# dfm/emcee

Hardware: NVIDIA H100
Metric: walker-steps/sec (nwalkers x iters / s) (higher is better)
Workload: dtype f64

## Files before the change

emcee_b200/_lib.py:

```python

import ctypes as C
import os

import numpy as np

__all__ = ["lib", "Engine", "Chain", "EngineError", "device_count", "LIB_PATH", "EbMove", "DeviceRows", "DeviceArray"]

HERE = os.path.dirname(os.path.abspath(__file__))
LIB_PATH = os.environ.get("EMCEE_B200_LIB") or os.path.join(HERE, "libemcee_b200.so")

EB_OK = 0
EB_ERR_INVALID = -1
EB_ERR_CUDA = -2
EB_ERR_COMM = -3
EB_ERR_STATE = -4
EB_ERR_UNSUPPORTED = -5
EB_ERR_NOMEM = -6
EB_ERR_CALLBACK = -7
EB_ERR_NAN_LOGPROB = -10
EB_ERR_INF_PARAM = -11
EB_ERR_NAN_PARAM = -12
EB_ERR_FEW_WALKERS = -13
EB_ERR_NAN_INITIAL = -14
EB_ERR_SINGULAR = -15
# ... 150 lines not shown
    "eb_trace_best": (C.c_int, [C.c_void_p, _dp, _dp, C.POINTER(C.c_uint64), C.POINTER(C.c_uint64)]),
    "eb_reservoir_config": (C.c_int, [C.c_void_p, C.c_uint64, C.c_uint64]),
    "eb_reservoir_count": (C.c_int, [C.c_void_p, C.POINTER(C.c_uint64), C.POINTER(C.c_uint64)]),
    "eb_reservoir_read": (C.c_int, [C.c_void_p, _dp, _dp, C.POINTER(C.c_uint64), C.POINTER(C.c_int64)]),
    "eb_reservoir_read_to": (C.c_int, [C.c_void_p, C.c_void_p, C.c_void_p, C.POINTER(C.c_uint64),
                                       C.POINTER(C.c_int64)]),
    "eb_walkers_gram": (C.c_int, [C.c_void_p, _dp, C.c_size_t, _dp, C.POINTER(C.c_int)]),
    "eb_autocorr": (C.c_int, [C.c_void_p, _dp, C.c_size_t, C.c_size_t, C.c_size_t, _dp]),
    "eb_last_step_timing": (C.c_int, [C.c_void_p, _dp, C.POINTER(C.c_uint64)]),
    "eb_debug_taps": (
        C.c_int,
        [C.c_void_p, C.POINTER(C.c_int64), _dp, _dp, C.POINTER(C.c_int64), C.POINTER(C.c_int64)],
    ),
    "eb_set_option": (C.c_int, [C.c_void_p, C.c_char_p, C.c_int64]),
    "eb_debug_timeline": (C.c_int, [C.c_void_p, C.POINTER(C.c_int64), C.c_size_t, C.POINTER(C.c_size_t)]),
    "eb_last_kernel_name": (C.c_char_p, [C.c_void_p]),
    "eb_last_kernel_variant": (C.c_char_p, [C.c_void_p]),
    "eb_microbench": (C.c_int, [C.c_int, C.c_int, _dp]),
    "eb_host_alloc": (C.c_int, [C.c_size_t, C.POINTER(C.c_void_p)]),
    "eb_host_free": (C.c_int, [C.c_void_p]),
    "eb_comm_id": (C.c_int, [C.c_char_p]),
    "eb_comm_init": (C.c_int, [C.c_void_p, C.c_char_p, C.c_int, C.c_int, C.c_int]),
    "eb_comm_export": (C.c_int, [C.c_void_p, C.c_char_p]),
    "eb_comm_import": (C.c_int, [C.c_void_p, C.c_char_p]),
    "eb_comm_probe": (C.c_int, [C.c_void_p, C.c_int, C.c_int, _dp]),
    "eb_device_alloc": (C.c_int, [C.c_int, C.c_size_t, C.POINTER(C.c_void_p)]),
    "eb_device_free": (C.c_int, [C.c_int, C.c_void_p]),
    "eb_device_copy": (C.c_int, [C.c_int, C.c_void_p, C.c_void_p, C.c_int64, C.c_int64, C.c_int64, C.c_uint64]),
    "eb_set_state_from": (C.c_int, [C.c_void_p, C.c_void_p, C.c_int64, C.c_void_p, C.c_int64, C.c_uint64]),
    "eb_get_state_to": (C.c_int, [C.c_void_p, C.c_void_p, C.c_void_p]),
# ... 1050 lines not shown
        self._check(
            lib().eb_debug_taps(
                self._h, partners.ctypes.data_as(i64), _as_dp(scalar), _as_dp(u),
                active.ctypes.data_as(i64), C.byref(cnt),
            )
        )
        k = int(cnt.value)
        return dict(partners=partners[:, :k], scalar=scalar[:k], u_accept=u[:k], active=active[:k])

    def debug_timeline(self):
        buf = np.zeros(1 << 21, dtype=np.int64)
        n = C.c_size_t()
        self._check(lib().eb_debug_timeline(self._h, buf.ctypes.data_as(C.POINTER(C.c_int64)), buf.size, C.byref(n)))
        return buf[: n.value].reshape(-1, 8, 8, 10)

    @staticmethod
    def comm_id():
        buf = C.create_string_buffer(EB_COMM_ID_BYTES)
        rc = lib().eb_comm_id(buf)
        if rc != EB_OK:
            raise EngineError("eb_comm_id failed (is libnccl.so.2 loadable?)")
        return buf.raw

    def comm_init(self, comm_id, rank, nranks, mode=EB_COMM_ALLGATHER):
        assert len(comm_id) == EB_COMM_ID_BYTES
        self._check(lib().eb_comm_init(self._h, comm_id, int(rank), int(nranks), int(mode)))

    def comm_export(self):
        buf = C.create_string_buffer(EB_IPC_BLOB_BYTES)
        self._check(lib().eb_comm_export(self._h, buf))
# ... 10 lines not shown
```

emcee_b200/csrc/capi.cu:

```cuda
#include <math.h>
#include <stdio.h>
#include <stdlib.h>
#include <string.h>

#include <algorithm>
#include <cmath>
#include <string>
#include <vector>

#include "chain_map.h"
#include "context.h"

static thread_local std::string g_create_err;

static const char* const MSG_BLOBS_WITH_LOG_PROB =
    "If you start sampling with a given log_prob, you also need to provide the current list of blobs at that "
    "position.";

int check_status(eb_ctx* c) {
  int f = *c->status_host;
  c->gm_unchecked = false;
  const unsigned long long g = graph_errors(c) ? *c->graph_err_host : 0ull;
  if (g != 0) {
    *c->graph_err_host = 0;
// ... 107 lines not shown
  cudaStream_t st = c->st.get();
  const size_t nd = (size_t)nwalkers * (size_t)ndim;
  CREATE_CK(dev_alloc(c->coords, nd * sizeof(double) + MAX_RANKS * sizeof(unsigned)));
  CREATE_CK(dev_alloc(c->logp, (size_t)nwalkers * sizeof(double)));
  CREATE_CK(dev_alloc(c->accepted, (size_t)nwalkers));
  CREATE_CK(dev_alloc(c->nacc, (size_t)nwalkers * sizeof(unsigned long long)));
  CREATE_CK(dev_alloc(c->status_dev, sizeof(int)));
  CREATE_CK(host_alloc(c->status_host, sizeof(int)));
  *c->status_host = 0;
  CREATE_CK(cudaMemsetAsync(c->status_dev.get(), 0, sizeof(int), st));
  CREATE_CK(cudaMemsetAsync(c->accepted.get(), 0, (size_t)nwalkers, st));
  CREATE_CK(cudaMemsetAsync(c->nacc.get(), 0, (size_t)nwalkers * sizeof(unsigned long long), st));
  size_t cap = (64u << 20) / ((size_t)nwalkers * sizeof(int32_t));
  cap = std::max<size_t>(1, std::min<size_t>(cap, 512));
  c->table_cap = cap;
  CREATE_CK(dev_alloc(c->order, cap * (size_t)nwalkers * sizeof(int32_t)));
  CREATE_CK(dev_alloc(c->info_dev, cap * sizeof(StepInfo)));
  CREATE_CK(host_alloc(c->info_host, cap * sizeof(StepInfo)));
  CREATE_CK(dev_alloc(c->descs_dev, cap * MAX_SPLITS * sizeof(HalfDesc)));
  CREATE_CK(host_alloc(c->descs_host, cap * MAX_SPLITS * sizeof(HalfDesc)));
  CREATE_CK(dev_alloc(c->gbar, sizeof(unsigned long long)));
  CREATE_CK(cudaMemsetAsync(c->gbar.get(), 0, sizeof(unsigned long long), st));
  CREATE_CK(cudaStreamSynchronize(st));
  *out = c.release();
  return EB_OK;
}

int eb_destroy(eb_ctx* c) {
  if (!c) return EB_OK;
  NOT_IN_CALLBACK(c);
// ... 1732 lines not shown
    c->local_first = (int)std::max<int64_t>(0, std::min<int64_t>(value, 2));
    return EB_OK;
  }
  if (!strcmp(name, "pdl")) {
    c->pdl = (int)std::max<int64_t>(0, std::min<int64_t>(value, 2));
    return EB_OK;
  }
  if (!strcmp(name, "moments_every")) {
    if (value < 0) FAIL(c, EB_ERR_INVALID, "moments_every must be >= 0");
    return moments_config(c, (uint64_t)value);
  }
  if (!strcmp(name, "tma_rows")) {
    c->allow_tma = (int)std::max<int64_t>(0, std::min<int64_t>(value, 2));
    return EB_OK;
  }
  if (!strcmp(name, "dense_dmma")) {
    c->allow_dmma = value != 0;
    return EB_OK;
  }
  FAIL(c, EB_ERR_INVALID, "eb_set_option: unknown option '%s'", name);
}

int eb_debug_timeline(eb_ctx* c, int64_t* out, size_t capacity, size_t* written) {
  if (!c || !out) return EB_ERR_INVALID;
  NOT_IN_CALLBACK(c);
  if (!c->timeline) FAIL(c, EB_ERR_STATE, "eb_debug_timeline: enable with eb_set_option(\"dmma_timeline\", 1)");
  CK(c, cudaSetDevice(c->device));
  const size_t n = (size_t)c->sm_count * 8 * TL_TILES * TL_EVENTS;
  if (capacity < n) FAIL(c, EB_ERR_INVALID, "eb_debug_timeline: need room for %zu values", n);
  CK(c, cudaMemcpy(out, c->timeline.get(), n * sizeof(long long), cudaMemcpyDeviceToHost));
// ... 167 lines not shown
```

emcee_b200/csrc/context.h:

```cpp
#pragma once

#include <stdio.h>

#include <string>
#include <vector>

#include "comm.h"
#include "engine.cuh"
#include "hist_bins.h"
#include "owners.h"
#include "reservoir_plan.h"
#include "trace_sum.h"

using namespace eb;


struct ChainSeg {
  DevPtr<double> x;
  DevPtr<double> lp;
};

struct eb_chain {
  int device = 0;
  int sm_count = 0;
// ... 30 lines not shown
  DevPtr<double> model_chol;
  DevPtr<double> model_box;
  bool have_model = false, have_state = false;

  DevPtr<int32_t> order;
  size_t table_cap = 0;
  DevPtr<StepInfo> info_dev;
  HostPtr<StepInfo> info_host;
  DevPtr<HalfDesc> descs_dev;
  HostPtr<HalfDesc> descs_host;
  DevPtr<unsigned long long> gbar;
  unsigned long long gbar_count = 0;
  uint64_t tbl_seed = 0, tbl_step0 = 0;
  size_t tbl_n = 0;
  std::vector<StepInfo> tbl_info;

  DevPtr<double> scratch_x;
  DevPtr<double> scratch_lp;
  size_t scratch_rows = 0;

  HostPtr<double> stage[2];
  HostPtr<uint8_t> stage_acc[2];
  EventPtr stage_ev[2];

  bool debug = false;
  DevPtr<int64_t> tap_partners;
  DevPtr<double> tap_scalar;
  DevPtr<double> tap_u;
  DevPtr<int64_t> tap_active;
  int64_t tap_count = 0;
// ... 170 lines not shown
      cudaGetLastError();                   \
      FAIL(ctx, EB_ERR_NOMEM, __VA_ARGS__); \
    }                                       \
  } while (0)

inline bool graph_mode(const eb_ctx* c) { return c->model.kind == MODEL_EXTERNAL && c->cb_where == EB_CALLBACK_GRAPH; }
inline bool proposal_graphs(const eb_ctx* c) {
  for (const eb_ctx::ProposalGraphs& p : c->prop_graphs)
    if (!p.graphs.empty()) return true;
  return false;
}
inline const eb_ctx::ProposalGraphs* slot_graphs(const eb_ctx* c, size_t slot) {
  return slot < c->prop_graphs.size() && !c->prop_graphs[slot].graphs.empty() ? &c->prop_graphs[slot] : nullptr;
}
inline bool graph_errors(const eb_ctx* c) { return graph_mode(c) || proposal_graphs(c); }
int check_status(eb_ctx* c);
int fetch_status(eb_ctx* c);
int enqueue_status_read(eb_ctx* c);
int run_callback(eb_ctx* c, const double* x, int64_t m, double* lp, bool scan_x);
void owned_rows(const eb_ctx* c, int64_t& r0, int64_t& r1);
int sync_replicas(eb_ctx* c);
```

emcee_b200/csrc/dense_dmma.cu:

```cuda
#include <math.h>

#include "draws.cuh"
#include "engine.cuh"
#include "tma.cuh"

namespace eb {

namespace {

constexpr int DMMA_CONSUMERS = 8;
constexpr int DMMA_THREADS = 64 * DMMA_CONSUMERS;
constexpr int NI = 2;
constexpr int DMMA_PRODUCER_REGS = 64;
constexpr int DMMA_CONSUMER_REGS = 192;
static_assert((DMMA_THREADS / 2) * (DMMA_PRODUCER_REGS + DMMA_CONSUMER_REGS) <= 65536, "register file of one SM");
__host__ __device__ constexpr bool dmma_rebalance(int KB, bool HAS_MEAN, bool BOUNDED) {
  return !BOUNDED && (KB >= 15 || (HAS_MEAN && KB >= 11));
}

__device__ __forceinline__ void dmma1688(double (&c)[4], double2 a01, double2 a23, double b0, double b1) {
  asm volatile(
      "mma.sync.aligned.m16n8k8.row.col.f64.f64.f64.f64 {%0,%1,%2,%3}, {%4,%5,%6,%7}, {%8,%9}, {%0,%1,%2,%3};"
      : "+d"(c[0]), "+d"(c[1]), "+d"(c[2]), "+d"(c[3])
      : "d"(a01.x), "d"(a01.y), "d"(a23.x), "d"(a23.y), "d"(b0), "d"(b1));
// ... 116 lines not shown
  double* sL = reinterpret_cast<double*>(smem_raw);
  double* sMu = sL + SL::off_mu;
  double* sSlots = sL + SL::off_slots;
  TileMeta* sMeta = reinterpret_cast<TileMeta*>(sL + SL::off_meta);
  uint64_t* bars = reinterpret_cast<uint64_t*>(smem_raw + SL::off_bars_bytes);
  volatile int* sAbort = reinterpret_cast<volatile int*>(smem_raw + SL::off_abort_bytes);
  volatile int* sPeers = sAbort + 1;
  int32_t* sInbox = reinterpret_cast<int32_t*>(smem_raw + SL::off_inbox_bytes);
  uint64_t* barL = bars;
  uint64_t* barFull = bars + 1;
  uint64_t* barReady = bars + 1 + DMMA_CONSUMERS;
  uint64_t* barFree = bars + 1 + 2 * DMMA_CONSUMERS;

  const int tid = threadIdx.x, lane = tid & 31, warp = tid >> 5;
  const bool is_producer = warp >= DMMA_CONSUMERS;
  const int pair = is_producer ? warp - DMMA_CONSUMERS : warp;
  const int g = lane >> 2, t = lane & 3;

  if (tid == 0) {
    *sAbort = 0;
    *sPeers = 0;
    mbar_init(barL, 1);
    for (int c = 0; c < DMMA_CONSUMERS; ++c) {
      mbar_init(barFull + c, 1);
      mbar_init(barReady + c, 1);
      mbar_init(barFree + c, 1);
    }
    asm volatile("fence.mbarrier_init.release.cluster;" ::: "memory");
  }
  if (HAS_MEAN)
    for (int k = tid; k < D; k += DMMA_THREADS) sMu[k] = a.model.params[k];
  __syncthreads();

  const int tstride = (int)gridDim.x * DMMA_CONSUMERS;
  const int tile0 = (int)blockIdx.x + (int)gridDim.x * pair;
  double* slot = sSlots + (size_t)pair * SL::slot_doubles;
  double* myS = slot + (size_t)g * RS + 2 * t;
  double* myC = myS + 8 * RS;
  TileMeta* meta = sMeta + 2 * pair;
  const bool multi = a.p2p_peer_flags != nullptr;
  unsigned k = 0;

  constexpr bool REBALANCE = dmma_rebalance(KB, HAS_MEAN, BOUNDED);
  if (is_producer) {
    if constexpr (REBALANCE) asm volatile("setmaxnreg.dec.sync.aligned.u32 %0;" ::"n"(DMMA_PRODUCER_REGS));
    const long long t_entry_p = clock64();
    long long* tlp = (TIMELINE && lane == 0)
                         ? a.timeline + ((size_t)blockIdx.x * DMMA_CONSUMERS + pair) * TL_TILES * TL_EVENTS : nullptr;
    const double dm1 = (double)a.D - 1.0;
    const int row = lane & 7;
    struct Prep {
      int32_t w, wp;
      double zz, factor, log_u, lp_old;
      bool valid, remote;
    };
    for (int h = 0; h < nhalf; ++h) {
      const HalfDesc d = (h == 0) ? d0 : descs[h];
      const int32_t* order = a.order + (size_t)d.order_step * a.N;
      const int2 rg = a.range ? a.range[(size_t)d.order_step * MAX_SPLITS + d.split] : make_int2(0, d.a_count);
      const int i_lo = rg.x, i_hi = rg.y;
      const int ntiles = (int)(((int64_t)i_hi - i_lo + 7) >> 3);
      const int64_t Nc = a.N - d.a_count;
      const int32_t* aperm = a.aperm ? a.aperm + (size_t)d.order_step * a.N + d.a_start : nullptr;
      auto prep = [&](int tile, bool with_lp) -> Prep {
        Prep p;
        int i = i_lo + tile * 8 + row;
        p.valid = i < i_hi;
        if (!p.valid) i = i_hi - 1;
        if (aperm) i = __ldg(aperm + i);
        const u32x4 A = prop_a(a.seed, d.step, (uint32_t)d.split, (uint32_t)i);
        p.zz = stretch_zz(A, a.p0);
        const int64_t r = stretch_rank(A, Nc);
        p.w = __ldg(order + d.a_start + i);
        p.wp = __ldg(order + complement_slot(r, d.a_start, d.a_count));
        p.log_u = log(accept_uniform(a.seed, d.step, (uint32_t)d.split, (uint32_t)i));
        p.factor = stretch_factor(dm1, p.zz);
        p.lp_old = with_lp ? a.logp[p.w] : 0.0;
        p.remote = multi && (p.wp / a.rows_per_rank != a.p2p_rank);
        return p;
      };
      auto peers_ready = [&]() -> bool {
        if (!multi || *sPeers > h) return true;
        if (pair == 0) {
          if (!peer_wait(a.p2p_my_flags, a.p2p_rank, a.p2p_nranks, a.p2p_wait + (unsigned)h, lane, a.status)) {
            *sAbort = 1;
            return false;
          }
          __syncwarp();
          if (lane == 0) *sPeers = h + 1;
        } else {
          while (*sPeers <= h) {
// ... 5 lines not shown
        return true;
      };
      auto request = [&](const Prep& p, int lo, int hi) {
        if (lane >= lo && lane < hi) {
          const bool partner = lane >= 8;
          const int32_t wr = partner ? p.wp : p.w;
          const double* base =
              (partner && a.peer_coords != nullptr) ? a.peer_coords[wr / a.rows_per_rank] : a.coords;
          bulk_g2s(slot + (size_t)(partner ? 8 : 0) * RS + (size_t)row * RS, base + (size_t)wr * D,
                   (unsigned)(D * sizeof(double)), barFull + pair);
        }
      };
      auto publish = [&](const Prep& p, int par) {
        TileMeta* m = meta + par;
        if (lane < 8) {
          m->factor[row] = p.factor;
          m->log_u[row] = p.log_u;
          m->lp_old[row] = p.lp_old;
          m->w[row] = p.valid ? p.w : -1;
        }
      };
      auto issue = [&](Prep& p, int par, bool load_lp) -> bool {
        if (__any_sync(0xffffffffu, p.remote) && !peers_ready()) return false;
        if (lane == 0) mbar_arrive_expect_tx(barFull + pair, 16u * D * (unsigned)sizeof(double));
        __syncwarp();
        request(p, 0, 16);
        if (load_lp) p.lp_old = a.logp[p.w];
        publish(p, par);
        return true;
      };
      Prep cur{}, nxt{};
      const bool early = h == 0 && a.dmma_early_own && tile0 < ntiles;
// ... 73 lines not shown
        if (tlq) tlq[8] = clock64() - t_entry_p;
        if (tile + tstride < ntiles) {
          cur = nxt;
          if (!mbar_wait_abortable(barFree + pair, k & 1u, sAbort)) return;
          if (tlq && (tile - tile0) / tstride + 1 < TL_TILES)
            tlq[TL_EVENTS + 6] = clock64() - t_entry_p;
          if (!issue(cur, (int)((k + 1) & 1u), h > 0 && tile == tile0)) return;
          if (tile + 2 * tstride < ntiles) nxt = prep(tile + 2 * tstride, true);
        }
      }
    }
    return;
  }

  if constexpr (REBALANCE) asm volatile("setmaxnreg.inc.sync.aligned.u32 %0;" ::"n"(DMMA_CONSUMER_REGS));
  if (tid == 0) {
    constexpr unsigned bytes = (unsigned)(SL::L_doubles * sizeof(double));
    mbar_arrive_expect_tx(barL, bytes);
    bulk_g2s(sL, a.model.chol, bytes, barL);
  }
  const long long t_entry = clock64();
  long long* tl = TIMELINE ? a.timeline + ((size_t)blockIdx.x * DMMA_CONSUMERS + pair) * TL_TILES * TL_EVENTS : nullptr;
  pdl_wait();
  pdl_launch_dependents();
  bool alive = mbar_wait_abortable_notrap(barL, 0, sAbort, a.status, FLAG_WAIT_TIMEOUT);
  for (int h = 0; h < nhalf; ++h) {
    const HalfDesc d = (h == 0) ? d0 : descs[h];
    const int2 rg = a.range ? a.range[(size_t)d.order_step * MAX_SPLITS + d.split] : make_int2(0, d.a_count);
    const int ntiles = (int)(((int64_t)rg.y - rg.x + 7) >> 3);
    unsigned kk = 0;
// ... 79 lines not shown
  if (multi) {
    __threadfence_system();
    asm volatile("bar.sync 1, %0;" ::"r"(32 * DMMA_CONSUMERS) : "memory");
    if (tid == 0 && !*sAbort) {
      const unsigned prev = atomicAdd(a.p2p_done, 1u);
      if (prev == gridDim.x - 1) {
        *a.p2p_done = 0;
        __threadfence_system();
        for (int r = 0; r < a.p2p_nranks; ++r)
          if (r != a.p2p_rank)
            atomicExch_system(a.p2p_peer_flags[r] + a.p2p_rank, a.p2p_signal + (unsigned)(nhalf - 1));
      }
    }
  }
}

template <int KB, bool HAS_MEAN>
__global__ void __launch_bounds__(256) logprob_dense_dmma_kernel(const ModelDev m, const double* __restrict__ x,
                                                                 const int64_t rows, double* __restrict__ out,
                                                                 int* status) {
  constexpr int D = 8 * KB;
  extern __shared__ __align__(16) unsigned char smem_raw[];
  double* sL = reinterpret_cast<double*>(smem_raw);
  double* sMu = sL + factor_doubles(KB);
  uint64_t* barL = reinterpret_cast<uint64_t*>(sMu + D);
  const int tid = threadIdx.x, lane = tid & 31, warp = tid >> 5;
  const int g = lane >> 2, t = lane & 3;
  if (tid == 0) {
    mbar_init(barL, 1);
    asm volatile("fence.mbarrier_init.release.cluster;" ::: "memory");
// ... 195 lines not shown
```

emcee_b200/csrc/engine.cuh:

```cuda
#pragma once
#include <cuda_runtime.h>
#include <stdint.h>

#include <string>
#include <vector>

#include "../../include/emcee_b200.h"
#include "acf_grid.h"
#include "philox.cuh"

namespace eb {

constexpr int MAX_SPLITS = 32;
constexpr int TABLE_THREADS = 1024;
constexpr int TL_TILES = 8, TL_EVENTS = 10;

enum : int {
  FLAG_NAN_LOGPROB = 1,
  FLAG_INF_PARAM = 2,
  FLAG_NAN_PARAM = 4,
  FLAG_COMM_TIMEOUT = 8,
  FLAG_WAIT_TIMEOUT = 16,
  FLAG_NAN_INITIAL = 32,
  FLAG_KDE_SINGULAR = 64,
};

struct ModelDev {
  int kind;
  const double* params;
  const double* chol;
  double s0, s1;
  const double* lo;
  const double* hi;
};

struct StepInfo {
  int32_t nsplits;
  int32_t randomize;
};

struct HalfStepArgs {
  double* coords;
  double* logp;
  uint8_t* accepted;
  unsigned long long* nacc;
  int* status;
  const int32_t* order;
  const double* const* peer_coords;
  int64_t rows_per_rank;
  unsigned* const* p2p_peer_flags;
  const unsigned* p2p_my_flags;
  unsigned* p2p_done;
  int p2p_rank, p2p_nranks;
  unsigned p2p_wait, p2p_signal;
// ... 4 lines not shown
  int split;
  int a_start, a_count;
  int i_lo, i_hi;
  const int2* range;
  const int32_t* aperm;
  int c_start[3], c_count[3];
  uint64_t seed, step;
  double p0, p1;
  ModelDev model;
  int64_t* tap_partners;
  double* tap_scalar;
  double* tap_u;
  int64_t* tap_active;
  long long* timeline;
  const double* qbuf;
};

constexpr int MOVE_PRECOMPUTED = 100;

constexpr int MODEL_EXTERNAL = 100;
struct ExternalBufs {
  double* q;
  double* f;
  const double* lp;
};

cudaError_t launch_split_tables(int32_t* order, const StepInfo* info_dev, int nsteps_chunk, int64_t N,
                                uint64_t seed, uint64_t step0, int64_t w_lo, int64_t w_hi, int2* ranges,
                                cudaStream_t st);
cudaError_t launch_locality_tables(const int32_t* order, const StepInfo* info_dev, const int2* ranges, int nsteps_chunk,
// ... 44 lines not shown
};
cudaError_t launch_half_step_tma(int move_kind, const HalfStepArgs& a, int sm_count, bool long_rows, bool own_reg,
                                 cudaStream_t st, bool* used, TmaVariant* variant = nullptr);
cudaError_t launch_logprob_generic(const ModelDev& m, const double* x, int64_t rows, int D, double* out,
                                   int* status, cudaStream_t st);
bool dense_dmma_supported(int D);
size_t dense_dmma_factor_doubles(int D);
void dense_dmma_pack_factor(const double* L, int D, double* packed);
cudaError_t launch_logprob_dense_dmma(const ModelDev& m, int D, const double* x, int64_t rows, double* out,
                                      int* status, int sm_count, cudaStream_t st);
struct HalfDesc {
  uint64_t step;
  int32_t order_step;
  int32_t split;
  int32_t a_start, a_count;
};
cudaError_t launch_dense_dmma(const HalfStepArgs& a, const HalfDesc& d0, const HalfDesc* descs_dev, int nhalf,
                              int max_count,
                              unsigned long long* gbar, unsigned long long gbar_base, int sm_count, bool pdl,
                              int* grid_out, cudaStream_t st);

cudaError_t launch_cov_chol(const double* acc, double n, int D, double* cov, double* L, cudaStream_t st);
cudaError_t launch_walk_shared_propose(const HalfStepArgs& a, const double* L, double* qbuf, cudaStream_t st);
bool walk_subset_supported(int D, int s0);
cudaError_t launch_walk_subset_propose(const HalfStepArgs& a, int s0, double* qbuf, cudaStream_t st);
cudaError_t launch_gaussian_shift(const double* L, int D, double f, uint64_t seed, uint64_t step, double* v,
                                  cudaStream_t st);
cudaError_t launch_gaussian_propose(const double* x0, int64_t row0, int64_t nrows, int D, int form, const double* scale,
                                    double f, int mode, int seq_dim, uint64_t seed, uint64_t step, double* qbuf,
                                    cudaStream_t st);

// ... 132 lines not shown
```

emcee_b200/csrc/kernels.cu:

```cuda
#include <math.h>

#include <algorithm>

#include "draws.cuh"
#include "engine.cuh"
#include "rowops.cuh"

namespace eb {

__global__ void __launch_bounds__(TABLE_THREADS) split_table_kernel(int32_t* __restrict__ order_base,
                                                                    const StepInfo* __restrict__ info,
                                                                    int64_t N, uint64_t seed,
                                                                    uint64_t step0, int64_t w_lo, int64_t w_hi,
                                                                    int2* __restrict__ ranges) {
  __shared__ int base[MAX_SPLITS];
  __shared__ int own_lo[MAX_SPLITS], own_hi[MAX_SPLITS];
  __shared__ int chunk_tot[MAX_SPLITS];
  __shared__ int warp_off[MAX_SPLITS][32];

  const int tid = threadIdx.x, lane = tid & 31, warp = tid >> 5;
  const uint64_t step = step0 + blockIdx.x;
  const int P = info[blockIdx.x].nsplits;
  const bool randomize = info[blockIdx.x].randomize != 0;
  int32_t* order = order_base + (size_t)blockIdx.x * (size_t)N;
// ... 41 lines not shown
      if (lane == 31) chunk_tot[warp] = incl;
    }
    __syncthreads();
    if (valid) order[base[sid] + warp_off[sid][warp] + my_prefix] = (int32_t)w;
    __syncthreads();
    if (tid < P) base[tid] += chunk_tot[tid];
    __syncthreads();
  }
  if (ranges != nullptr && tid < P) ranges[(size_t)blockIdx.x * MAX_SPLITS + tid] = make_int2(own_lo[tid], own_hi[tid]);
}

cudaError_t launch_split_tables(int32_t* order, const StepInfo* info_dev, int nsteps_chunk, int64_t N,
                                uint64_t seed, uint64_t step0, int64_t w_lo, int64_t w_hi, int2* ranges,
                                cudaStream_t st) {
  split_table_kernel<<<nsteps_chunk, TABLE_THREADS, 0, st>>>(order, info_dev, N, seed, step0, w_lo, w_hi, ranges);
  return cudaGetLastError();
}

__global__ void __launch_bounds__(TABLE_THREADS) locality_table_kernel(const int32_t* __restrict__ order_base,
                                                                       const StepInfo* __restrict__ info,
                                                                       const int2* __restrict__ ranges, int64_t N,
                                                                       uint64_t seed, uint64_t step0,
                                                                       int64_t rows_per_rank, int rank, int front_cap,
                                                                       int32_t* __restrict__ aperm_base) {
  __shared__ int warp_cnt[2][32], loc_cnt[32];
  __shared__ int base_sh[2], nfront_sh, seen_local_sh;
  const int tid = threadIdx.x, lane = tid & 31, warp = tid >> 5;
  const int P = info[blockIdx.x].nsplits, split = blockIdx.y;
  if (split >= P) return;
  const uint64_t step = step0 + blockIdx.x;
// ... 403 lines not shown
```

emcee_b200/csrc/step.cu:

```cuda
#include <math.h>
#include <stdarg.h>
#include <stdio.h>
#include <string.h>

#include <algorithm>
#include <cmath>
#include <vector>

#include "context.h"

namespace {

struct Schedule {
  std::vector<eb_move> moves;
  std::vector<double> cdf;
  std::vector<int> gform;
  std::vector<size_t> goff;
};

void chol_psd_host(const double* A, int D, std::vector<double>& L) {
  L.assign((size_t)D * D, 0.0);
  double m = 0.0;
  for (int j = 0; j < D; ++j) m = std::max(m, A[(size_t)j * D + j]);
  const double tol = 1e-12 * m;
// ... 642 lines not shown
struct DmmaGroup {
  size_t first = 0;
  int nhalf = 0;
  int max_count = 0;
};

struct DmmaChain {
  bool live = false;
  HalfDesc first{}, last{};
};

int flush_dmma(eb_ctx* c, const eb_move& mv, DmmaGroup& grp, DmmaChain& chain, uint64_t& launches) {
  if (grp.nhalf == 0) return EB_OK;
  HalfStepArgs a = move_args(c, mv);
  a.order = c->order.get();
  a.range = c->comm.nranks > 1 ? c->comm.ranges : nullptr;
  int bound = grp.max_count;
  if (c->comm.nranks > 1 && c->comm.rows_per_rank < bound) bound = (int)c->comm.rows_per_rank;
  const bool few_tiles = (bound + 7) / 8 <= 2 * DMMA_TILE_SLOTS * c->sm_count;
  a.aperm = (c->comm.nranks > 1 && (c->local_first == 2 || (c->local_first == 1 && few_tiles))) ? c->comm.aperm : nullptr;
  const bool fused = comm_fuse_barrier(c->comm, a, grp.nhalf);
  c->fused_last = fused;
  const bool pdl = chain.live && grp.nhalf == 1 && (c->comm.nranks > 1 ? c->pdl >= 2 : c->pdl >= 1);
  const HalfDesc& d0 = c->descs_host.get()[grp.first];
  a.dmma_early_own = pdl && c->comm.nranks == 1 && d0.split > 0 && chain.first.step == d0.step &&
                     chain.first.order_step == d0.order_step && chain.last.step == d0.step &&
                     chain.last.split == d0.split - 1;
  if (c->timeline_first_split && d0.split != 0) a.timeline = nullptr;
  int grid = 0;
  CK(c, launch_dense_dmma(a, c->descs_host.get()[grp.first], c->descs_dev.get() + grp.first, grp.nhalf, bound,
// ... 2 lines not shown
  c->dmma_nhalf_max = std::max(c->dmma_nhalf_max, grp.nhalf);
  note_kernel(c, "dense_dmma", "dense_dmma nhalf_max=%d grid=%d", c->dmma_nhalf_max, grid);
  chain.live = grid > 0;
  chain.first = c->descs_host.get()[grp.first];
  chain.last = c->descs_host.get()[grp.first + grp.nhalf - 1];
  ++launches;
  grp = DmmaGroup{};
  return EB_OK;
}

struct Chunk {
  std::vector<size_t> pick;
  size_t off = 0;
  size_t build = 0;
  size_t ndesc = 0;
};

int prepare_chunk(eb_ctx* c, const Schedule& s, size_t n, Chunk& ch) {
  CK(c, cudaStreamSynchronize(c->st.get()));
  ch.pick.resize(n);
  for (size_t k = 0; k < n; ++k) {
    ch.pick[k] = choose_move(c, s, c->step + k);
    const eb_move& mv = s.moves[ch.pick[k]];
    c->info_host.get()[k].nsplits = mv.nsplits;
    c->info_host.get()[k].randomize = mv.randomize_split;
  }
  ch.off = 0;
  ch.build = 0;
  bool hit = c->tbl_n > 0 && c->tbl_seed == c->seed && c->step >= c->tbl_step0 && c->step + n <= c->tbl_step0 + c->tbl_n;
  if (hit) {
    ch.off = (size_t)(c->step - c->tbl_step0);
    for (size_t k = 0; k < n && hit; ++k)
      hit = c->tbl_info[ch.off + k].nsplits == c->info_host.get()[k].nsplits &&
            c->tbl_info[ch.off + k].randomize == c->info_host.get()[k].randomize;
  }
  if (!hit) {
    ch.off = 0;
    ch.build = std::min<size_t>(c->table_cap, std::max<size_t>(n, 64));
    for (size_t k = n; k < ch.build; ++k) {
      const eb_move& mv = s.moves[choose_move(c, s, c->step + k)];
      c->info_host.get()[k].nsplits = mv.nsplits;
      c->info_host.get()[k].randomize = mv.randomize_split;
    }
    c->tbl_seed = c->seed;
    c->tbl_step0 = c->step;
    c->tbl_n = ch.build;
    c->tbl_info.assign(c->info_host.get(), c->info_host.get() + ch.build);
  }
  ch.ndesc = 0;
  for (size_t k = 0; k < n; ++k) {
    const eb_move& mv = s.moves[ch.pick[k]];
    if (!dmma_eligible(c, mv)) continue;
    int start[MAX_SPLITS + 1];
    split_starts(c->N, mv.nsplits, start);
    for (int split = 0; split < mv.nsplits; ++split) {
      HalfDesc& d = c->descs_host.get()[ch.ndesc++];
      d.step = c->step + k;
      d.order_step = (int32_t)(ch.off + k);
      d.split = split;
      d.a_start = start[split];
      d.a_count = start[split + 1] - start[split];
    }
  }
  return EB_OK;
}

int upload_chunk(eb_ctx* c, const Chunk& ch, uint64_t& launches) {
  if (ch.ndesc)
    CK(c, cudaMemcpyAsync(c->descs_dev.get(), c->descs_host.get(), ch.ndesc * sizeof(HalfDesc), cudaMemcpyHostToDevice,
                          c->st.get()));
  if (ch.build) {
    CK(c, cudaMemcpyAsync(c->info_dev.get(), c->info_host.get(), ch.build * sizeof(StepInfo), cudaMemcpyHostToDevice,
                          c->st.get()));
    const Comm& cm = c->comm;
    CK(c, launch_split_tables(c->order.get(), c->info_dev.get(), (int)ch.build, c->N, c->seed, c->step,
                              cm.rows_per_rank * cm.rank, cm.rows_per_rank * (cm.rank + 1),
                              cm.nranks > 1 ? cm.ranges : nullptr, c->st.get()));
    ++launches;
    if (cm.nranks > 1 && cm.aperm) {
      CK(c, launch_locality_tables(c->order.get(), c->info_dev.get(), cm.ranges, (int)ch.build, c->N, c->seed,
                                   c->step, cm.rows_per_rank, cm.rank, 64 * c->sm_count, cm.aperm, c->st.get()));
      ++launches;
    }
  }
  return EB_OK;
}

int reserve_trace(eb_ctx* c, uint64_t nsteps);
unsigned stats_due(const eb_ctx* c, uint64_t n);
int accumulate_due(eb_ctx* c, unsigned due, uint64_t& launches);

struct GraphRun {
  eb_ctx* c;
  explicit GraphRun(eb_ctx* ctx) : c(ctx) {
    c->graph_run = graph_errors(c);
    c->graph_step0 = c->step;
    c->graph_picks.clear();
  }
  ~GraphRun() { c->graph_run = false; }
// ... 14 lines not shown
    }
  }
  if (c->trace_every > 0) {
    const int rc = reserve_trace(c, nsteps);
    if (rc) return rc;
  }
  c->dmma_nhalf_max = 0;
  CK(c, cudaEventRecord(c->ev0.get(), c->st.get()));
  if (comm_begin(c->comm, c->st.get(), c->status_dev.get(), launches)) FAIL(c, EB_ERR_COMM, "%s", c->comm.err.c_str());
  c->fused_last = false;
  const bool multi = c->comm.nranks > 1;
  const bool one_per_launch = multi;
  const bool exchange_each = multi && c->comm.mode == EB_COMM_ALLGATHER;
  DmmaChain chain;
  Chunk ch;
  uint64_t done = 0;
  while (done < nsteps) {
    const size_t chunk = (size_t)std::min<uint64_t>(nsteps - done, c->table_cap);
    int rc = EB_OK;
    if (c->graph_run && done > 0) rc = fetch_status(c);
    if (!rc) rc = prepare_chunk(c, s, chunk, ch);
    if (rc) return rc;
    DmmaGroup grp;
    size_t desc_cursor = 0;
    const eb_move* grp_move = nullptr;
    for (size_t k = 0; k < chunk; ++k) {
      const eb_move& mv = s.moves[ch.pick[k]];
      if (c->gm_unchecked && !graph_mode(c) && !captured_proposal(c, mv)) {
        rc = fetch_status(c);
        if (rc) return rc;
      }
      const unsigned due = stats_due(c, c->step + 1);
      const bool stored = sync_every > 0 && (done + k + 1) % sync_every == 0;
      if (perstep) {
        CK(c, cudaMemsetAsync(c->flush_buf.get(), (int)(k & 0xff), c->flush_bytes, c->st.get()));
        CK(c, cudaEventRecord(c->ev_pool[2 * (done + k)].get(), c->st.get()));
// ... 184 lines not shown
  if (!rc && (due & STAT_RESERVOIR)) rc = accumulate_reservoir(c, launches);
  return rc;
}

int step_preflight(eb_ctx* c) {
  if (!c->have_model) FAIL(c, EB_ERR_STATE, "eb_step: no model set");
  if (!c->have_state) FAIL(c, EB_ERR_STATE, "eb_step: no state set");
  CK(c, cudaSetDevice(c->device));
  return EB_OK;
}

}

extern "C" {

int eb_step(eb_ctx* c, const eb_move* moves, size_t nmoves, uint64_t nsteps, uint8_t* accepted_last) {
  if (!c) return EB_ERR_INVALID;
  NOT_IN_CALLBACK(c);
  int rc = step_preflight(c);
  if (rc) return rc;
  Schedule s;
  rc = build_schedule(c, moves, nmoves, s);
  if (rc) return rc;
  if (nsteps > 0) {
    rc = run_steps(c, s, nsteps, 0, [](uint64_t) { return EB_OK; });
    if (rc) return rc;
  }
  if (accepted_last) {
    rc = sync_replicas(c);
    if (rc) return rc;
// ... 128 lines not shown
```

include/emcee_b200.h:

```cpp
#ifndef EMCEE_B200_H
#define EMCEE_B200_H

#include <stddef.h>
#include <stdint.h>

#ifdef __cplusplus
extern "C" {
#endif

#define EB_ABI_VERSION 2

typedef enum eb_status {
  EB_OK = 0,
  EB_ERR_INVALID = -1,
  EB_ERR_CUDA = -2,
  EB_ERR_COMM = -3,
  EB_ERR_STATE = -4,
  EB_ERR_UNSUPPORTED = -5,
  EB_ERR_NOMEM = -6,
  EB_ERR_CALLBACK = -7,
  EB_ERR_NAN_LOGPROB = -10,
  EB_ERR_INF_PARAM = -11,
  EB_ERR_NAN_PARAM = -12,
  EB_ERR_FEW_WALKERS = -13,
// ... 173 lines not shown
int eb_trace_config(eb_ctx* ctx, uint64_t every);
int eb_trace_count(eb_ctx* ctx, uint64_t* rows);
int eb_trace_read(eb_ctx* ctx, uint64_t first, uint64_t count, uint64_t* step, double* rows_out);
int eb_trace_best(eb_ctx* ctx, double* coords, double* log_prob, uint64_t* step, uint64_t* walker);
int eb_reservoir_config(eb_ctx* ctx, uint64_t size, uint64_t every);
int eb_reservoir_count(eb_ctx* ctx, uint64_t* offered, uint64_t* kept);
int eb_reservoir_read(eb_ctx* ctx, double* coords, double* log_prob, uint64_t* step, int64_t* walker);
int eb_reservoir_read_to(eb_ctx* ctx, double* coords_dst, double* log_prob_dst, uint64_t* step, int64_t* walker);
int eb_walkers_gram(eb_ctx* ctx, const double* coords, size_t rows, double* gram, int* flags);
int eb_autocorr(eb_ctx* ctx, const double* chain, size_t n_step, size_t n_walker, size_t n_param, double* acf);

int eb_last_step_timing(const eb_ctx* ctx, double* ms, uint64_t* launches);
int eb_debug_taps(eb_ctx* ctx, int64_t* partners, double* scalar, double* u_accept,
                  int64_t* active, int64_t* nactive);
int eb_debug_timeline(eb_ctx* ctx, int64_t* out, size_t capacity, size_t* written);
int eb_set_option(eb_ctx* ctx, const char* name, int64_t value);
const char* eb_last_kernel_name(const eb_ctx* ctx);
const char* eb_last_kernel_variant(const eb_ctx* ctx);

int eb_microbench(int what, int warps_per_sm, double* result);
int eb_host_alloc(size_t bytes, void** out);
int eb_host_free(void* ptr);

#define EB_COMM_ID_BYTES 128
int eb_comm_id(char id[EB_COMM_ID_BYTES]);
#define EB_COMM_ALLGATHER 0
#define EB_COMM_P2P 1
int eb_comm_init(eb_ctx* ctx, const char id[EB_COMM_ID_BYTES], int rank, int nranks, int mode);
#define EB_IPC_BLOB_BYTES 256
int eb_comm_export(eb_ctx* ctx, char blob[EB_IPC_BLOB_BYTES]);
// ... 9 lines not shown
```

Baseline: 947.2 million.

## Precompute stretch-move draws into a per-chunk plan buffer for the DMMA kernel

Adds a separate kernel that, before each chunk of dense DMMA steps, computes the stretch-move draws (zz, factor, log_u, walker and partner indices) and writes them to a 32-byte-per-record device plan. The DMMA producer warp then reads these with vectorized loads instead of computing Philox-style draws, a log, and two dependent order lookups inline. This takes RNG and index arithmetic off the producer's critical path. The cost is an extra kernel launch per chunk, extra global memory traffic and a plan buffer, and chunk size may now be capped by plan capacity. Table building also now sizes itself on the remaining steps rather than the current chunk.

```diff
diff --git a/emcee_b200/_lib.py b/emcee_b200/_lib.py
--- a/emcee_b200/_lib.py
+++ b/emcee_b200/_lib.py
@@ -188,6 +188,10 @@
     ),
     "eb_set_option": (C.c_int, [C.c_void_p, C.c_char_p, C.c_int64]),
     "eb_debug_timeline": (C.c_int, [C.c_void_p, C.POINTER(C.c_int64), C.c_size_t, C.POINTER(C.c_size_t)]),
+    "eb_debug_stretch_plan": (
+        C.c_int,
+        [C.c_void_p, C.c_uint64, C.c_int64, C.c_int, C.c_int, C.c_double, C.c_int64, C.c_int64, C.c_void_p, C.c_size_t],
+    ),
     "eb_last_kernel_name": (C.c_char_p, [C.c_void_p]),
     "eb_last_kernel_variant": (C.c_char_p, [C.c_void_p]),
     "eb_microbench": (C.c_int, [C.c_int, C.c_int, _dp]),
@@ -1268,6 +1272,19 @@
         self._check(lib().eb_debug_timeline(self._h, buf.ctypes.data_as(C.POINTER(C.c_int64)), buf.size, C.byref(n)))
         return buf[: n.value].reshape(-1, 8, 8, 10)
 
+    STRETCH_DRAW = np.dtype([("zz", "<f8"), ("w", "<i4"), ("wp", "<i4"), ("factor", "<f8"), ("log_u", "<f8")])
+
+    def debug_stretch_plan(self, step0, nsteps, nsplits, randomize, a, w_range=None):
+        out = np.zeros((int(nsteps), self.nwalkers), dtype=self.STRETCH_DRAW)
+        lo, hi = (-1, -1) if w_range is None else (int(w_range[0]), int(w_range[1]))
+        self._check(
+            lib().eb_debug_stretch_plan(
+                self._h, int(step0), int(nsteps), int(nsplits), int(bool(randomize)), float(a), lo, hi,
+                out.ctypes.data_as(C.c_void_p), out.nbytes,
+            )
+        )
+        return out
+
     @staticmethod
     def comm_id():
         buf = C.create_string_buffer(EB_COMM_ID_BYTES)
diff --git a/emcee_b200/csrc/capi.cu b/emcee_b200/csrc/capi.cu
--- a/emcee_b200/csrc/capi.cu
+++ b/emcee_b200/csrc/capi.cu
@@ -145,6 +145,7 @@
   size_t cap = (64u << 20) / ((size_t)nwalkers * sizeof(int32_t));
   cap = std::max<size_t>(1, std::min<size_t>(cap, 512));
   c->table_cap = cap;
+  c->plan_cap = plan_cap_default(c.get());
   CREATE_CK(dev_alloc(c->order, cap * (size_t)nwalkers * sizeof(int32_t)));
   CREATE_CK(dev_alloc(c->info_dev, cap * sizeof(StepInfo)));
   CREATE_CK(host_alloc(c->info_host, cap * sizeof(StepInfo)));
@@ -1907,6 +1908,17 @@
     c->allow_tma = (int)std::max<int64_t>(0, std::min<int64_t>(value, 2));
     return EB_OK;
   }
+  if (!strcmp(name, "dmma_plan_steps")) {
+    if (value < 0) FAIL(c, EB_ERR_INVALID, "dmma_plan_steps must be >= 0");
+    const size_t cap = value == 0 ? plan_cap_default(c) : std::min<size_t>((size_t)value, plan_cap_default(c));
+    if (cap != c->plan_cap) {
+      CK(c, cudaSetDevice(c->device));
+      CK(c, cudaStreamSynchronize(c->st.get()));
+      c->plan.reset();
+      c->plan_cap = cap;
+    }
+    return EB_OK;
+  }
   if (!strcmp(name, "dense_dmma")) {
     c->allow_dmma = value != 0;
     return EB_OK;
diff --git a/emcee_b200/csrc/context.h b/emcee_b200/csrc/context.h
--- a/emcee_b200/csrc/context.h
+++ b/emcee_b200/csrc/context.h
@@ -2,6 +2,7 @@
 
 #include <stdio.h>
 
+#include <algorithm>
 #include <string>
 #include <vector>
 
@@ -68,6 +69,8 @@
   uint64_t tbl_seed = 0, tbl_step0 = 0;
   size_t tbl_n = 0;
   std::vector<StepInfo> tbl_info;
+  DevPtr<StretchDraw> plan;
+  size_t plan_cap = 0;
 
   DevPtr<double> scratch_x;
   DevPtr<double> scratch_lp;
@@ -268,6 +271,10 @@
   return slot < c->prop_graphs.size() && !c->prop_graphs[slot].graphs.empty() ? &c->prop_graphs[slot] : nullptr;
 }
 inline bool graph_errors(const eb_ctx* c) { return graph_mode(c) || proposal_graphs(c); }
+inline size_t plan_cap_default(const eb_ctx* c) {
+  const size_t cap = (64u << 20) / ((size_t)c->N * sizeof(StretchDraw));
+  return std::max<size_t>(1, std::min<size_t>(cap, c->table_cap));
+}
 int check_status(eb_ctx* c);
 int fetch_status(eb_ctx* c);
 int enqueue_status_read(eb_ctx* c);
diff --git a/emcee_b200/csrc/dense_dmma.cu b/emcee_b200/csrc/dense_dmma.cu
--- a/emcee_b200/csrc/dense_dmma.cu
+++ b/emcee_b200/csrc/dense_dmma.cu
@@ -154,7 +154,6 @@
 
   const int tid = threadIdx.x, lane = tid & 31, warp = tid >> 5;
   const bool is_producer = warp >= DMMA_CONSUMERS;
-  const int pair = is_producer ? warp - DMMA_CONSUMERS : warp;
   const int g = lane >> 2, t = lane & 3;
 
   if (tid == 0) {
@@ -172,11 +171,13 @@
     for (int k = tid; k < D; k += DMMA_THREADS) sMu[k] = a.model.params[k];
   __syncthreads();
 
-  const int tstride = (int)gridDim.x * DMMA_CONSUMERS;
-  const int tile0 = (int)blockIdx.x + (int)gridDim.x * pair;
-  double* slot = sSlots + (size_t)pair * SL::slot_doubles;
-  double* myS = slot + (size_t)g * RS + 2 * t;
-  double* myC = myS + 8 * RS;
+#define EB_DMMA_PAIR_LAYOUT(PAIR)                                                            \
+  const int pair = (PAIR);                                                                   \
+  const int tstride = (int)gridDim.x * DMMA_CONSUMERS;                                       \
+  const int tile0 = (int)blockIdx.x + (int)gridDim.x * pair;              \
+  double* slot = sSlots + (size_t)pair * SL::slot_doubles;                                   \
+  double* myS = slot + (size_t)g * RS + 2 * t;      \
+  double* myC = myS + 8 * RS;                           \
   TileMeta* meta = sMeta + 2 * pair;
   const bool multi = a.p2p_peer_flags != nullptr;
   unsigned k = 0;
@@ -184,23 +185,22 @@
   constexpr bool REBALANCE = dmma_rebalance(KB, HAS_MEAN, BOUNDED);
   if (is_producer) {
     if constexpr (REBALANCE) asm volatile("setmaxnreg.dec.sync.aligned.u32 %0;" ::"n"(DMMA_PRODUCER_REGS));
+    EB_DMMA_PAIR_LAYOUT(warp - DMMA_CONSUMERS)
     const long long t_entry_p = clock64();
     long long* tlp = (TIMELINE && lane == 0)
                          ? a.timeline + ((size_t)blockIdx.x * DMMA_CONSUMERS + pair) * TL_TILES * TL_EVENTS : nullptr;
-    const double dm1 = (double)a.D - 1.0;
     const int row = lane & 7;
     struct Prep {
-      int32_t w, wp;
-      double zz, factor, log_u, lp_old;
+      int32_t i, w, wp;
+      double zz, lp_old;
       bool valid, remote;
     };
     for (int h = 0; h < nhalf; ++h) {
       const HalfDesc d = (h == 0) ? d0 : descs[h];
-      const int32_t* order = a.order + (size_t)d.order_step * a.N;
       const int2 rg = a.range ? a.range[(size_t)d.order_step * MAX_SPLITS + d.split] : make_int2(0, d.a_count);
       const int i_lo = rg.x, i_hi = rg.y;
       const int ntiles = (int)(((int64_t)i_hi - i_lo + 7) >> 3);
-      const int64_t Nc = a.N - d.a_count;
+      const StretchDraw* plan = a.plan + (size_t)d.plan_step * a.N + d.a_start;
       const int32_t* aperm = a.aperm ? a.aperm + (size_t)d.order_step * a.N + d.a_start : nullptr;
       auto prep = [&](int tile, bool with_lp) -> Prep {
         Prep p;
@@ -208,13 +208,11 @@
         p.valid = i < i_hi;
         if (!p.valid) i = i_hi - 1;
         if (aperm) i = __ldg(aperm + i);
-        const u32x4 A = prop_a(a.seed, d.step, (uint32_t)d.split, (uint32_t)i);
-        p.zz = stretch_zz(A, a.p0);
-        const int64_t r = stretch_rank(A, Nc);
-        p.w = __ldg(order + d.a_start + i);
-        p.wp = __ldg(order + complement_slot(r, d.a_start, d.a_count));
-        p.log_u = log(accept_uniform(a.seed, d.step, (uint32_t)d.split, (uint32_t)i));
-        p.factor = stretch_factor(dm1, p.zz);
+        const int4 r = __ldg(reinterpret_cast<const int4*>(plan + i));
+        p.i = i;
+        p.zz = __hiloint2double(r.y, r.x);
+        p.w = r.z;
+        p.wp = r.w;
         p.lp_old = with_lp ? a.logp[p.w] : 0.0;
         p.remote = multi && (p.wp / a.rows_per_rank != a.p2p_rank);
         return p;
@@ -250,8 +248,9 @@
       auto publish = [&](const Prep& p, int par) {
         TileMeta* m = meta + par;
         if (lane < 8) {
-          m->factor[row] = p.factor;
-          m->log_u[row] = p.log_u;
+          const double2 fu = __ldg(reinterpret_cast<const double2*>(plan + p.i) + 1);
+          m->factor[row] = fu.x;
+          m->log_u[row] = fu.y;
           m->lp_old[row] = p.lp_old;
           m->w[row] = p.valid ? p.w : -1;
         }
@@ -355,6 +354,7 @@
   }
 
   if constexpr (REBALANCE) asm volatile("setmaxnreg.inc.sync.aligned.u32 %0;" ::"n"(DMMA_CONSUMER_REGS));
+  EB_DMMA_PAIR_LAYOUT(warp)
   if (tid == 0) {
     constexpr unsigned bytes = (unsigned)(SL::L_doubles * sizeof(double));
     mbar_arrive_expect_tx(barL, bytes);
@@ -464,6 +464,8 @@
     }
   }
 }
+
+#undef EB_DMMA_PAIR_LAYOUT
 
 template <int KB, bool HAS_MEAN>
 __global__ void __launch_bounds__(256) logprob_dense_dmma_kernel(const ModelDev m, const double* __restrict__ x,
diff --git a/emcee_b200/csrc/engine.cuh b/emcee_b200/csrc/engine.cuh
--- a/emcee_b200/csrc/engine.cuh
+++ b/emcee_b200/csrc/engine.cuh
@@ -38,6 +38,15 @@
   int32_t nsplits;
   int32_t randomize;
 };
+
+struct alignas(16) StretchDraw {
+  double zz;
+  int32_t w;
+  int32_t wp;
+  double factor;
+  double log_u;
+};
+static_assert(sizeof(StretchDraw) == 32, "two 16-byte loads per record");
 
 struct HalfStepArgs {
   double* coords;
@@ -72,6 +81,7 @@
   int64_t* tap_active;
   long long* timeline;
   const double* qbuf;
+  const StretchDraw* plan;
 };
 
 constexpr int MOVE_PRECOMPUTED = 100;
@@ -146,7 +156,11 @@
   int32_t order_step;
   int32_t split;
   int32_t a_start, a_count;
-};
+  int32_t plan_step;
+  double a;
+};
+cudaError_t launch_stretch_plan(StretchDraw* plan, const int32_t* order, const HalfDesc* descs_dev, int ndesc,
+                                int max_count, const int2* ranges, int64_t N, int D, uint64_t seed, cudaStream_t st);
 cudaError_t launch_dense_dmma(const HalfStepArgs& a, const HalfDesc& d0, const HalfDesc* descs_dev, int nhalf,
                               int max_count,
                               unsigned long long* gbar, unsigned long long gbar_base, int sm_count, bool pdl,
diff --git a/emcee_b200/csrc/kernels.cu b/emcee_b200/csrc/kernels.cu
--- a/emcee_b200/csrc/kernels.cu
+++ b/emcee_b200/csrc/kernels.cu
@@ -79,6 +79,34 @@
                                 uint64_t seed, uint64_t step0, int64_t w_lo, int64_t w_hi, int2* ranges,
                                 cudaStream_t st) {
   split_table_kernel<<<nsteps_chunk, TABLE_THREADS, 0, st>>>(order, info_dev, N, seed, step0, w_lo, w_hi, ranges);
+  return cudaGetLastError();
+}
+
+__global__ void __launch_bounds__(256) stretch_plan_kernel(StretchDraw* __restrict__ plan,
+                                                           const int32_t* __restrict__ order_base,
+                                                           const HalfDesc* __restrict__ descs,
+                                                           const int2* __restrict__ ranges, int64_t N, double dm1,
+                                                           uint64_t seed) {
+  const HalfDesc d = descs[blockIdx.y];
+  const int2 rg = ranges ? ranges[(size_t)d.order_step * MAX_SPLITS + d.split] : make_int2(0, d.a_count);
+  const int64_t i = (int64_t)rg.x + (int64_t)blockIdx.x * blockDim.x + threadIdx.x;
+  if (i >= rg.y) return;
+  const int32_t* order = order_base + (size_t)d.order_step * N;
+  const u32x4 A = prop_a(seed, d.step, (uint32_t)d.split, (uint32_t)i);
+  StretchDraw r;
+  r.zz = stretch_zz(A, d.a);
+  r.factor = stretch_factor(dm1, r.zz);
+  r.log_u = log(accept_uniform(seed, d.step, (uint32_t)d.split, (uint32_t)i));
+  r.w = order[d.a_start + i];
+  r.wp = order[complement_slot(stretch_rank(A, N - d.a_count), d.a_start, d.a_count)];
+  plan[(size_t)d.plan_step * N + d.a_start + i] = r;
+}
+
+cudaError_t launch_stretch_plan(StretchDraw* plan, const int32_t* order, const HalfDesc* descs_dev, int ndesc,
+                                int max_count, const int2* ranges, int64_t N, int D, uint64_t seed, cudaStream_t st) {
+  if (ndesc <= 0 || max_count <= 0) return cudaSuccess;
+  const dim3 grid((unsigned)((max_count + 255) / 256), (unsigned)ndesc);
+  stretch_plan_kernel<<<grid, 256, 0, st>>>(plan, order, descs_dev, ranges, N, (double)D - 1.0, seed);
   return cudaGetLastError();
 }
 
diff --git a/emcee_b200/csrc/step.cu b/emcee_b200/csrc/step.cu
--- a/emcee_b200/csrc/step.cu
+++ b/emcee_b200/csrc/step.cu
@@ -680,6 +680,7 @@
   if (grp.nhalf == 0) return EB_OK;
   HalfStepArgs a = move_args(c, mv);
   a.order = c->order.get();
+  a.plan = c->plan.get();
   a.range = c->comm.nranks > 1 ? c->comm.ranges : nullptr;
   int bound = grp.max_count;
   if (c->comm.nranks > 1 && c->comm.rows_per_rank < bound) bound = (int)c->comm.rows_per_rank;
@@ -712,9 +713,33 @@
   size_t off = 0;
   size_t build = 0;
   size_t ndesc = 0;
+  int max_count = 0;
 };
 
-int prepare_chunk(eb_ctx* c, const Schedule& s, size_t n, Chunk& ch) {
+int dmma_descs(const eb_ctx* c, const eb_move& mv, uint64_t step, int order_step, int plan_step, HalfDesc* out) {
+  int start[MAX_SPLITS + 1];
+  split_starts(c->N, mv.nsplits, start);
+  for (int split = 0; split < mv.nsplits; ++split) {
+    HalfDesc& d = out[split];
+    d.step = step;
+    d.order_step = order_step;
+    d.split = split;
+    d.a_start = start[split];
+    d.a_count = start[split + 1] - start[split];
+    d.plan_step = plan_step;
+    d.a = mv.p0;
+  }
+  return mv.nsplits;
+}
+
+int build_stretch_plan(eb_ctx* c, int ndesc, int max_count, const int2* ranges) {
+  if (!c->plan) CK(c, dev_alloc(c->plan, c->plan_cap * (size_t)c->N * sizeof(StretchDraw)));
+  CK(c, launch_stretch_plan(c->plan.get(), c->order.get(), c->descs_dev.get(), ndesc, max_count, ranges, c->N, c->D,
+                            c->seed, c->st.get()));
+  return EB_OK;
+}
+
+int prepare_chunk(eb_ctx* c, const Schedule& s, size_t n, uint64_t left, Chunk& ch) {
   CK(c, cudaStreamSynchronize(c->st.get()));
   ch.pick.resize(n);
   for (size_t k = 0; k < n; ++k) {
@@ -734,7 +759,7 @@
   }
   if (!hit) {
     ch.off = 0;
-    ch.build = std::min<size_t>(c->table_cap, std::max<size_t>(n, 64));
+    ch.build = (size_t)std::min<uint64_t>(c->table_cap, std::max<uint64_t>(left, 64));
     for (size_t k = n; k < ch.build; ++k) {
       const eb_move& mv = s.moves[choose_move(c, s, c->step + k)];
       c->info_host.get()[k].nsplits = mv.nsplits;
@@ -746,19 +771,13 @@
     c->tbl_info.assign(c->info_host.get(), c->info_host.get() + ch.build);
   }
   ch.ndesc = 0;
+  ch.max_count = 0;
   for (size_t k = 0; k < n; ++k) {
     const eb_move& mv = s.moves[ch.pick[k]];
     if (!dmma_eligible(c, mv)) continue;
-    int start[MAX_SPLITS + 1];
-    split_starts(c->N, mv.nsplits, start);
-    for (int split = 0; split < mv.nsplits; ++split) {
-      HalfDesc& d = c->descs_host.get()[ch.ndesc++];
-      d.step = c->step + k;
-      d.order_step = (int32_t)(ch.off + k);
-      d.split = split;
-      d.a_start = start[split];
-      d.a_count = start[split + 1] - start[split];
-    }
+    HalfDesc* d = c->descs_host.get() + ch.ndesc;
+    ch.ndesc += dmma_descs(c, mv, c->step + k, (int)(ch.off + k), (int)k, d);
+    ch.max_count = std::max(ch.max_count, (int)d[0].a_count);
   }
   return EB_OK;
 }
@@ -781,6 +800,10 @@
       ++launches;
     }
   }
+  if (ch.ndesc) {
+    const int rc = build_stretch_plan(c, (int)ch.ndesc, ch.max_count, c->comm.nranks > 1 ? c->comm.ranges : nullptr);
+    if (rc) return rc;
+  }
   return EB_OK;
 }
 
@@ -825,12 +848,15 @@
   const bool exchange_each = multi && c->comm.mode == EB_COMM_ALLGATHER;
   DmmaChain chain;
   Chunk ch;
+  size_t chunk_cap = c->table_cap;
+  for (const eb_move& mv : s.moves)
+    if (dmma_eligible(c, mv)) chunk_cap = std::min(chunk_cap, c->plan_cap);
   uint64_t done = 0;
   while (done < nsteps) {
-    const size_t chunk = (size_t)std::min<uint64_t>(nsteps - done, c->table_cap);
+    const size_t chunk = (size_t)std::min<uint64_t>(nsteps - done, chunk_cap);
     int rc = EB_OK;
     if (c->graph_run && done > 0) rc = fetch_status(c);
-    if (!rc) rc = prepare_chunk(c, s, chunk, ch);
+    if (!rc) rc = prepare_chunk(c, s, chunk, nsteps - done, ch);
     if (rc) return rc;
     DmmaGroup grp;
     size_t desc_cursor = 0;
@@ -1045,6 +1071,49 @@
 
 extern "C" {
 
+int eb_debug_stretch_plan(eb_ctx* c, uint64_t step0, int64_t nsteps, int nsplits, int randomize, double a, int64_t w_lo,
+                          int64_t w_hi, void* out, size_t capacity) {
+  if (!c || !out) return EB_ERR_INVALID;
+  NOT_IN_CALLBACK(c);
+  if (nsteps < 1 || (size_t)nsteps > c->plan_cap)
+    FAIL(c, EB_ERR_INVALID, "eb_debug_stretch_plan: nsteps must be in [1, %zu]", c->plan_cap);
+  if (nsplits < 2 || nsplits > MAX_SPLITS) FAIL(c, EB_ERR_INVALID, "eb_debug_stretch_plan: nsplits must be in [2, 32]");
+  const bool sharded = w_lo >= 0;
+  if (sharded && !(w_lo <= w_hi && w_hi <= c->N)) FAIL(c, EB_ERR_INVALID, "eb_debug_stretch_plan: bad walker range");
+  const size_t bytes = (size_t)nsteps * (size_t)c->N * sizeof(StretchDraw);
+  if (capacity < bytes) FAIL(c, EB_ERR_INVALID, "eb_debug_stretch_plan: need room for %zu bytes", bytes);
+  CK(c, cudaSetDevice(c->device));
+  cudaStream_t st = c->st.get();
+  CK(c, cudaStreamSynchronize(st));
+  DevPtr<int2> ranges;
+  if (sharded) CK(c, dev_alloc(ranges, (size_t)nsteps * MAX_SPLITS * sizeof(int2)));
+  if (!c->plan) CK(c, dev_alloc(c->plan, c->plan_cap * (size_t)c->N * sizeof(StretchDraw)));
+  eb_move mv{};
+  mv.kind = EB_MOVE_STRETCH;
+  mv.nsplits = nsplits;
+  mv.randomize_split = randomize;
+  mv.p0 = a;
+  size_t ndesc = 0;
+  int max_count = 0;
+  for (int64_t k = 0; k < nsteps; ++k) {
+    c->info_host.get()[k] = StepInfo{nsplits, randomize};
+    HalfDesc* d = c->descs_host.get() + ndesc;
+    ndesc += dmma_descs(c, mv, step0 + (uint64_t)k, (int)k, (int)k, d);
+    max_count = std::max(max_count, (int)d[0].a_count);
+  }
+  c->tbl_n = 0;
+  CK(c, cudaMemcpyAsync(c->info_dev.get(), c->info_host.get(), nsteps * sizeof(StepInfo), cudaMemcpyHostToDevice, st));
+  CK(c, launch_split_tables(c->order.get(), c->info_dev.get(), (int)nsteps, c->N, c->seed, step0, sharded ? w_lo : 0,
+                            sharded ? w_hi : c->N, ranges.get(), st));
+  CK(c, cudaMemcpyAsync(c->descs_dev.get(), c->descs_host.get(), ndesc * sizeof(HalfDesc), cudaMemcpyHostToDevice, st));
+  CK(c, cudaMemsetAsync(c->plan.get(), 0, bytes, st));
+  const int rc = build_stretch_plan(c, (int)ndesc, max_count, ranges.get());
+  if (rc) return rc;
+  CK(c, cudaMemcpyAsync(out, c->plan.get(), bytes, cudaMemcpyDeviceToHost, st));
+  CK(c, cudaStreamSynchronize(st));
+  return EB_OK;
+}
+
 int eb_step(eb_ctx* c, const eb_move* moves, size_t nmoves, uint64_t nsteps, uint8_t* accepted_last) {
   if (!c) return EB_ERR_INVALID;
   NOT_IN_CALLBACK(c);
diff --git a/include/emcee_b200.h b/include/emcee_b200.h
--- a/include/emcee_b200.h
+++ b/include/emcee_b200.h
@@ -211,6 +211,8 @@
 int eb_debug_taps(eb_ctx* ctx, int64_t* partners, double* scalar, double* u_accept,
                   int64_t* active, int64_t* nactive);
 int eb_debug_timeline(eb_ctx* ctx, int64_t* out, size_t capacity, size_t* written);
+int eb_debug_stretch_plan(eb_ctx* ctx, uint64_t step0, int64_t nsteps, int nsplits, int randomize, double a,
+                          int64_t w_lo, int64_t w_hi, void* out, size_t capacity);
 int eb_set_option(eb_ctx* ctx, const char* name, int64_t value);
 const char* eb_last_kernel_name(const eb_ctx* ctx);
 const char* eb_last_kernel_variant(const eb_ctx* ctx);
```

Result: no change. 950.2 million, median of 6 (+0.3%).
